# alanqrwang/nwhead

Hardware: AMD Instinct MI355X
Metric: query-predictions/sec (higher is better)
Workload: dtype f32; 1 GPU; K3 predict('full'): B=256 queries/step vs bank N=50000 d=512 C=200, bank sharded 1-way, 26 query batches coalesced per launch; B=256, N_support=50000, d=512, C=200, parallelism=support-shard x1

## Files before the change

### nwhead_amd/csrc/fused.hip

```cpp
#include <mutex>
#include <utility>
#include <vector>
#include "fused_impl.h"

namespace nw {

#define NW_EXTERN_FUSED_KIND(K) extern template int launch_fused_kind<K>(const FusedArgs&, const FusedPlan&);
NW_FOR_EACH_KIND(NW_EXTERN_FUSED_KIND)
#undef NW_EXTERN_FUSED_KIND

namespace {
struct TileTimer {
    bool on = false;
    std::vector<std::pair<hipEvent_t, hipEvent_t>> ev;
    std::vector<std::pair<hipEvent_t, hipEvent_t>> pool;
    std::mutex mu;
} g_tt;
}

int tile_timer_start(hipStream_t st) {
    if (!g_tt.on) return -1;
    std::lock_guard<std::mutex> lk(g_tt.mu);
    std::pair<hipEvent_t, hipEvent_t> p;
    if (!g_tt.pool.empty()) {
        p = g_tt.pool.back();
        g_tt.pool.pop_back();
    } else if (hipEventCreate(&p.first) != hipSuccess || hipEventCreate(&p.second) != hipSuccess) {
        return -1;
    }
    (void)hipEventRecord(p.first, st);
    g_tt.ev.push_back(p);
    return (int)g_tt.ev.size() - 1;
}
void tile_timer_stop(int slot, hipStream_t st) {
    if (slot < 0) return;
    std::lock_guard<std::mutex> lk(g_tt.mu);
    if (slot < (int)g_tt.ev.size()) (void)hipEventRecord(g_tt.ev[slot].second, st);
}
int tile_timer_enable(bool on) {
    std::lock_guard<std::mutex> lk(g_tt.mu);
    g_tt.on = on;
    return NW_OK;
}
int tile_timer_read(double* total_us, int64_t* launches) {
    std::lock_guard<std::mutex> lk(g_tt.mu);
    double tot = 0;
    for (auto& p : g_tt.ev) {
        float ms = 0.f;
        if (hipEventSynchronize(p.second) != hipSuccess || hipEventElapsedTime(&ms, p.first, p.second) != hipSuccess)
            return NW_ERR_LAUNCH;
        tot += (double)ms * 1e3;
        g_tt.pool.push_back(p);
    }
    if (total_us) *total_us = tot;
    if (launches) *launches = (int64_t)g_tt.ev.size();
    g_tt.ev.clear();
    return NW_OK;
}

namespace {
int device_cu_count() {
    static int n = [] {
        int dev = 0, v = 0;
        if (hipGetDevice(&dev) != hipSuccess) return 256;
        if (hipDeviceGetAttribute(&v, hipDeviceAttributeMultiprocessorCount, dev) != hipSuccess || v <= 0) return 256;
        return v;
    }();
    return n;
}
bool env_flag(int k) { return knob(k) == 1; }
}

inline size_t al256(size_t x) { return (x + 255) & ~(size_t)255; }

size_t fused_layout(int64_t B, int64_t n_stiles, int BS, char* base, FusedWs* ws, int64_t C) {
    size_t off = 0;
    auto take = [&](size_t bytes) {
        char* p = base ? base + off : nullptr;
        off += al256(bytes);
        return p;
    };
    FusedWs w;
    w.m = reinterpret_cast<float*>(take((size_t)n_stiles * B * 4));
    w.den = reinterpret_cast<float*>(take((size_t)n_stiles * B * 4));
    w.nrun = reinterpret_cast<int*>(take((size_t)n_stiles * 4));
    w.lab = reinterpret_cast<int*>(take((size_t)n_stiles * BS * 4));
    w.num = reinterpret_cast<float*>(take((size_t)n_stiles * BS * B * 4));
    w.runid = reinterpret_cast<int*>(take(((size_t)n_stiles * BS + 64) * 4));
    w.bnd = reinterpret_cast<int*>(take((size_t)n_stiles * 2 * 4));
    w.ctab = reinterpret_cast<int*>(take((size_t)C * (3 + 4) * 4));
    if (ws) *ws = w;
    return off;
}

namespace {

constexpr int MTHREADS = 512, MENT = 4, MTPT = 16;
template <bool PARTIAL, int MQ, int TMODE>
__global__ __launch_bounds__(MTHREADS) void nw_merge_runs_kernel(
    const float* __restrict__ ws_m, const float* __restrict__ ws_den, const int* __restrict__ ws_nrun,
    const int* __restrict__ ws_lab, const float* __restrict__ ws_num, float* __restrict__ out,
    float* __restrict__ lse, float* __restrict__ m_out, float* __restrict__ den_out,
    float* __restrict__ num_out, int B, int C, int n_stiles, int BS, const int* __restrict__ ctab) {
    constexpr bool TABLES = TMODE != 0;
    constexpr bool LTAB = TMODE == 1;
    constexpr int ML = MTHREADS / MQ;
    constexpr int MNS = MQ + 1;
    constexpr int NW = MTHREADS / 64;
    constexpr float LN2 = 0.693147180559945309417f;
    static_assert(MQ <= 32 && (MQ & (MQ - 1)) == 0, "a wave holds whole groups of MQ queries");
    extern __shared__ __attribute__((aligned(16))) char smem[];
    float* red = reinterpret_cast<float*>(smem);
    float* Ms = red + 2 * NW * MQ;
    float* inv_s = Ms + MQ;
    int* lds_tab = reinterpret_cast<int*>(inv_s + MQ);
    int* cnt = TMODE == 2 ? const_cast<int*>(ctab) : lds_tab;
    int* tlo = cnt + C;
    int* thi = tlo + C;
    int* ent = thi + C;
    float* res = reinterpret_cast<float*>(lds_tab + (size_t)C * (3 + MENT));
    const int tid = threadIdx.x, bq = tid & (MQ - 1), sl = tid / MQ, wave = tid >> 6;
    const int b0 = blockIdx.x * MQ;
    const int b = min(b0 + bq, B - 1);

    const bool in_regs = n_stiles <= ML * MTPT;
    float mr[MTPT], dr[MTPT];
    float M = -INFINITY;
    if (in_regs) {
#pragma unroll
        for (int u = 0; u < MTPT; ++u) {
            const int t = sl + u * ML;
            const bool ok = t < n_stiles;
            mr[u] = ok ? ws_m[(size_t)t * B + b] : -INFINITY;
            dr[u] = ok ? ws_den[(size_t)t * B + b] : 0.f;
        }
    }
    int tnr = 0, tl3[3] = {-1, -1, -1};
    const bool one_pass_tables = LTAB && n_stiles <= MTHREADS;
    if (one_pass_tables && tid < n_stiles) {
        tnr = ws_nrun[tid];
        const int* lt = ws_lab + (size_t)tid * BS;
        tl3[0] = lt[0];
        tl3[1] = lt[1];
        tl3[2] = lt[2];
    }
    if (LTAB) {
        for (int c = tid; c < C; c += MTHREADS) {
            cnt[c] = 0;
            tlo[c] = 0x7fffffff;
            thi[c] = -1;
        }
    }
    if (in_regs) {
#pragma unroll
        for (int u = 0; u < MTPT; ++u) M = fmaxf(M, mr[u]);
    } else {
        for (int t = sl; t < n_stiles; t += ML) M = fmaxf(M, ws_m[(size_t)t * B + b]);
    }
#pragma unroll
    for (int o = 32; o >= MQ; o >>= 1) M = fmaxf(M, __shfl_xor(M, o));
    if ((tid & 63) < MQ) red[wave * MQ + bq] = M;
    __syncthreads();
    if (LTAB) {
        auto add_tile = [&](int t, int nr, const int (&l3)[3]) {
            const int* lt = ws_lab + (size_t)t * BS;
            for (int r = 0; r < nr; ++r) {
                const int y = r < 3 ? l3[r] : lt[r];
                if (y < 0) continue;
                atomicMin(&tlo[y], t);
                atomicMax(&thi[y], t);
                const int slot = atomicAdd(&cnt[y], 1);
                if (slot < MENT) ent[y * MENT + slot] = t * BS + r;
            }
        };
        if (one_pass_tables) {
            if (tid < n_stiles) add_tile(tid, tnr, tl3);
        } else {
            for (int t = tid; t < n_stiles; t += MTHREADS) {
                const int* lt = ws_lab + (size_t)t * BS;
                const int l3[3] = {lt[0], lt[1], lt[2]};
                add_tile(t, ws_nrun[t], l3);
            }
        }
    }
    M = red[bq];
#pragma unroll
    for (int k = 1; k < NW; ++k) M = fmaxf(M, red[k * MQ + bq]);
    float den = 0.f;
    if (in_regs) {
#pragma unroll
        for (int u = 0; u < MTPT; ++u) den += dr[u] * __builtin_amdgcn_exp2f(mr[u] - M);
    } else {
        for (int t = sl; t < n_stiles; t += ML)
            den += ws_den[(size_t)t * B + b] * __builtin_amdgcn_exp2f(ws_m[(size_t)t * B + b] - M);
    }
#pragma unroll
    for (int o = 32; o >= MQ; o >>= 1) den += __shfl_xor(den, o);
    if ((tid & 63) < MQ) red[NW * MQ + wave * MQ + bq] = den;
    if (sl == 0) Ms[bq] = M;
    __syncthreads();
    if (LTAB) {
        for (int c = tid; c < C; c += MTHREADS) {
            const int n = cnt[c];
            if (n > 1 && n <= MENT) {
                int e[MENT];
#pragma unroll
                for (int k = 0; k < MENT; ++k) e[k] = k < n ? ent[c * MENT + k] : 0x7fffffff;
#pragma unroll
                for (int i = 1; i < MENT; ++i)
#pragma unroll
                    for (int j = MENT - 1; j >= i; --j)
                        if (e[j] < e[j - 1]) { const int x = e[j]; e[j] = e[j - 1]; e[j - 1] = x; }
#pragma unroll
                for (int k = 0; k < MENT; ++k)
                    if (k < n) ent[c * MENT + k] = e[k];
            }
        }
    }
    den = red[NW * MQ + bq];
#pragma unroll
    for (int k = 1; k < NW; ++k) den += red[NW * MQ + k * MQ + bq];
    if (sl == 0) inv_s[bq] = 1.f / den;
    const int nq = min(MQ, B - b0);
    if (sl == 0 && bq < nq) {
        if (PARTIAL) {
            m_out[b] = M * LN2;
            den_out[b] = den;
        } else if (lse) {
            lse[b] = M * LN2 + logf(den);
        }
    }
    __syncthreads();
    int P = 1;
    while (P < 64 && 2 * P * C * MQ <= MTHREADS) P <<= 1;
    for (int xx = tid; xx < C * MQ * P; xx += MTHREADS) {
        const int x = xx / P, sub = xx - x * P;
        const int c = x / MQ, q = x - c * MQ;
        const int bb = min(b0 + q, B - 1);
        const float Mq = Ms[q];
        float acc = 0.f;
        const int n = TABLES ? cnt[c] : MENT + 1;
        if (n <= MENT) {
            int e[MENT];
            float v[MENT], mt[MENT];
#pragma unroll
            for (int k = 0; k < MENT; ++k) e[k] = ent[c * MENT + (k < n ? k : 0)];
#pragma unroll
            for (int k = 0; k < MENT; ++k) {
                if (k < n) {
                    v[k] = ws_num[(size_t)e[k] * B + bb];
                    mt[k] = ws_m[(size_t)(e[k] / BS) * B + bb];
                }
            }
#pragma unroll
            for (int k = 0; k < MENT; ++k)
                if (k < n) acc += v[k] * __builtin_amdgcn_exp2f(mt[k] - Mq);
        } else {
            const int t0 = TABLES ? tlo[c] : 0, t1 = TABLES ? thi[c] : n_stiles - 1;
            for (int t = t0 + sub; t <= t1; t += P) {
                const int nr = ws_nrun[t];
                const float f = __builtin_amdgcn_exp2f(ws_m[(size_t)t * B + bb] - Mq);
                const int* lt = ws_lab + (size_t)t * BS;
                for (int r = 0; r < nr; ++r)
                    if (lt[r] == c) acc += ws_num[((size_t)t * BS + r) * B + bb] * f;
            }
        }
        if (P > 1) {
            if (n <= MENT && sub != 0) acc = 0.f;
            for (int o = P >> 1; o > 0; o >>= 1) acc += __shfl_xor(acc, o);
            if (sub != 0) continue;
        }
        if (LTAB && MQ > 1) {
            res[c * MNS + q] = acc;
        } else if (q < nq) {
            if (PARTIAL) num_out[(size_t)bb * C + c] = acc;
            else out[(size_t)bb * C + c] = logf(acc * inv_s[q] + NW_LOG_EPS);
        }
    }
    if (!LTAB || MQ == 1) return;
    __syncthreads();
    for (int x = tid; x < nq * C; x += MTHREADS) {
        const int qq = x / C, c = x - qq * C;
        if (PARTIAL) num_out[(size_t)(b0 + qq) * C + c] = res[c * MNS + qq];
        else out[(size_t)(b0 + qq) * C + c] = logf(res[c * MNS + qq] * inv_s[qq] + NW_LOG_EPS);
    }
}

__global__ __launch_bounds__(1024) void nw_class_tables_kernel(const int* __restrict__ ws_nrun, const int* __restrict__ ws_lab,
                                                                int n_stiles, int BS, int C, int* __restrict__ ctab) {
    int* cnt = ctab;
    int* tlo = cnt + C;
    int* thi = tlo + C;
    int* ent = thi + C;
    const int tid = threadIdx.x;
    for (int c = tid; c < C; c += 1024) {
        cnt[c] = 0;
        tlo[c] = 0x7fffffff;
        thi[c] = -1;
    }
    __threadfence();
    __syncthreads();
    for (int t = tid; t < n_stiles; t += 1024) {
        const int nr = ws_nrun[t];
        const int* lt = ws_lab + (size_t)t * BS;
        for (int r = 0; r < nr; ++r) {
            const int y = lt[r];
            if (y < 0) continue;
            atomicMin(&tlo[y], t);
            atomicMax(&thi[y], t);
            const int slot = atomicAdd(&cnt[y], 1);
            if (slot < MENT) ent[y * MENT + slot] = t * BS + r;
        }
    }
    __threadfence();
    __syncthreads();
    for (int c = tid; c < C; c += 1024) {
        const int n = cnt[c];
        if (n > 1 && n <= MENT) {
            int e[MENT];
#pragma unroll
            for (int k = 0; k < MENT; ++k) e[k] = k < n ? ent[c * MENT + k] : 0x7fffffff;
#pragma unroll
            for (int i = 1; i < MENT; ++i)
#pragma unroll
                for (int j = MENT - 1; j >= i; --j)
                    if (e[j] < e[j - 1]) { const int x = e[j]; e[j] = e[j - 1]; e[j - 1] = x; }
#pragma unroll
            for (int k = 0; k < MENT; ++k)
                if (k < n) ent[c * MENT + k] = e[k];
        }
    }
}

__global__ __launch_bounds__(64) void nw_run_tables_kernel(const int64_t* __restrict__ sy, int N, int C, int BS,
                                                           int* __restrict__ runid, int* __restrict__ nrun,
                                                           int* __restrict__ lab_out, int* __restrict__ bnd) {
    const int st = blockIdx.x, lane = threadIdx.x, s0 = st * BS;
    if (lane < 2) bnd[2 * st + lane] = BS;
    __syncthreads();
    int lab[3], flag[3];
#pragma unroll
    for (int u = 0; u < 3; ++u) {
        const int t = 3 * lane + u, j = s0 + t;
        int64_t y = -1;
        if (t < BS && j < N) y = sy[j];
        lab[u] = ((uint64_t)y < (uint64_t)C) ? (int)y : -1;
    }
    const int prev_last = __shfl_up(lab[2], 1);
    flag[0] = (lane == 0) || (lab[0] != prev_last);
    flag[1] = lab[1] != lab[0];
    flag[2] = lab[2] != lab[1];
    int incl = flag[0] + flag[1] + flag[2];
#pragma unroll
    for (int o = 1; o < 64; o <<= 1) {
        const int v = __shfl_up(incl, o);
        if (lane >= o) incl += v;
    }
    int id = incl - (flag[0] + flag[1] + flag[2]) - 1;
#pragma unroll
    for (int u = 0; u < 3; ++u) {
        const int t = 3 * lane + u;
        id += flag[u];
        if (t < BS) {
            runid[(size_t)s0 + t] = id;
            if (flag[u]) lab_out[(size_t)s0 + id] = lab[u];
            if (flag[u] && (id == 1 || id == 2)) bnd[2 * st + id - 1] = t;
            if (t == BS - 1) nrun[st] = id + 1;
        }
    }
}

int env_rs() {
    const int v = knob(KNOB_TILE_RS);
    return v == KNOB_UNSET ? 0 : v;
}

}

int query_area_of_workspace(void* workspace, size_t workspace_bytes, int64_t B, int64_t N, int64_t d, int64_t C, float** rows,
                            float** scale, float** norm2) {
    const size_t total = nw_fwd_workspace_bytes(B, N, d, C);
    if (!workspace || workspace_bytes < total) return NW_ERR_WORKSPACE;
    const size_t a = al256((size_t)B * (size_t)d * sizeof(float)), b = al256((size_t)B * sizeof(float));
    char* base = static_cast<char*>(workspace) + (total - a - 3 * b);
    *rows = reinterpret_cast<float*>(base);
    *scale = reinterpret_cast<float*>(base + a);
    *norm2 = reinterpret_cast<float*>(base + a + b);
    return NW_OK;
}

int launch_run_tables(const FusedWs& ws, const int64_t* sy, int N, int C, int n_stiles, int BS, hipStream_t st) {
    if (BS > 192) return NW_ERR_UNSUPPORTED;
    hipLaunchKernelGGL(nw_run_tables_kernel, dim3(n_stiles), dim3(64), 0, st, sy, N, C, BS, ws.runid, ws.nrun, ws.lab, ws.bnd);
    NW_CHECK_LAUNCH();
    return NW_OK;
}

constexpr int BANK_BS = 128;

size_t bank_tables_layout(int64_t n_stiles, char* base, FusedWs* ws) {
    size_t off = 0;
    auto take = [&](size_t bytes) {
        char* p = base ? base + off : nullptr;
        off += al256(bytes);
        return p;
    };
    int* nrun = reinterpret_cast<int*>(take((size_t)n_stiles * 4));
    int* lab = reinterpret_cast<int*>(take((size_t)n_stiles * BANK_BS * 4));
    int* runid = reinterpret_cast<int*>(take(((size_t)n_stiles * BANK_BS + 64) * 4));
    int* bnd = reinterpret_cast<int*>(take((size_t)n_stiles * 2 * 4));
    if (ws) {
        ws->nrun = nrun;
        ws->lab = lab;
        ws->runid = runid;
        ws->bnd = bnd;
    }
    return off;
}

bool bank_tables_take(const int64_t* sy, int N, int C, int n_stiles, int BS, FusedWs* ws) {
    (void)C;
    const FwdOpts& o = fwd_opts();
    if (!o.tables || BS != BANK_BS) return false;
    if (o.tables_sy != sy || o.tables_N != (int64_t)N) return false;
    if (o.tables_bytes < bank_tables_layout(n_stiles, nullptr, nullptr)) return false;
    bank_tables_layout(n_stiles, const_cast<char*>(o.tables), ws);
    return true;
}

int launch_merge_runs(const FusedWs& ws, float* out, float* lse, float* m, float* den, float* num,
                      int B, int C, int n_stiles, int BS, hipStream_t st) {
    auto lds_bytes = [&](int mq, bool tables) {
        return ((size_t)2 * (MTHREADS / 64) * mq + 2 * mq + (tables ? (size_t)C * (3 + MENT + mq + 1) : 0)) * sizeof(float);
    };
    const size_t cap = 150 * 1024;
    int mq = 1;
    const int force_mq = knob(KNOB_MERGE_MQ) == KNOB_UNSET ? 0 : knob(KNOB_MERGE_MQ);
    if (force_mq == 1 || force_mq == 16 || force_mq == 32) {
        mq = force_mq;
        if (lds_bytes(mq, true) > cap) mq = 1;
    } else if (B >= 512 && !env_flag(KNOB_MERGE_PER_QUERY)) {
        mq = n_stiles >= 128 ? 16 : 32;
        if (lds_bytes(mq, true) > cap) mq = 16;
        if (lds_bytes(mq, true) > cap) mq = 1;
    }
    const bool tables = lds_bytes(mq, true) <= cap;
    const size_t lds = lds_bytes(mq, tables);
    const int grid = (B + mq - 1) / mq;
#define NW_MERGE(P_, Q_, T_)                                                                                       \
    hipLaunchKernelGGL((nw_merge_runs_kernel<P_, Q_, T_>), dim3(grid), dim3(MTHREADS), lds, st, ws.m, ws.den, ws.nrun, \
                       ws.lab, ws.num, out, lse, m, den, num, B, C, n_stiles, BS, ws.ctab)
    if (!tables) {
        if (ws.ctab && !env_flag(KNOB_MERGE_NO_GLOBAL_TABLES)) {
            hipLaunchKernelGGL(nw_class_tables_kernel, dim3(1), dim3(1024), 0, st, ws.nrun, ws.lab, n_stiles, BS, C, ws.ctab);
            if (out) NW_MERGE(false, 1, 2); else NW_MERGE(true, 1, 2);
        } else {
            if (out) NW_MERGE(false, 1, 0); else NW_MERGE(true, 1, 0);
        }
    } else if (mq == 1) {
        if (out) NW_MERGE(false, 1, 1); else NW_MERGE(true, 1, 1);
    } else if (mq == 16) {
        if (out) NW_MERGE(false, 16, 1); else NW_MERGE(true, 16, 1);
    } else {
        if (out) NW_MERGE(false, 32, 1); else NW_MERGE(true, 32, 1);
    }
#undef NW_MERGE
    NW_CHECK_LAUNCH();
    return NW_OK;
}

int pick_rs(int64_t B, int64_t N, int64_t d, bool f16) {
    const int forced = env_rs();
    if (forced == 2 || forced == 4 || forced == 5 || forced == 6 || forced == 8 || forced == 10 || forced == 12)
        return forced;
    const int64_t nq = (B + BQ - 1) / BQ;
    if (forced == 0 && !f16 && d % BK == 0 && nq * ((N + 79) / 80) >= 480) return 5;
    if (forced == 0 && f16 && d % BK == 0 && nq * ((N + 127) / 128) >= 4 * 256) return 8;
    const int cand[] = {2, 4, 6, 8, 10, 12};
    const int ncand = f16 ? 5 : 6;
    double best = 1e30;
    int best_rs = 8;
    for (int ci = 0; ci < ncand; ++ci) {
        const int rs = cand[ci];
        const int64_t ns = (N + 16 * rs - 1) / (16 * rs);
        const int64_t nwg = nq * ns;
        const int64_t rounds = (nwg + 255) / 256;
        double cost = (double)rounds * (rs + 1.5);
        if (nwg >= 384) cost *= 0.85;
        if (cost < best - 1e-9) {
            best = cost;
            best_rs = rs;
        }
    }
    return best_rs;
}

bool half_form_shape_ok(int64_t d) {
    return d % 64 == 0 && d >= 192 && d <= (1 << 20);
}

namespace {
struct TileLds {
    size_t reg, dma;
    size_t p64, p64x2, p128;
};
template <int RS>
constexpr TileLds tile_lds() {
    if constexpr (RS > 5)
        return {FUSED_HDR + TileCfg<RS>::STAGE_BYTES, FUSED_HDR + DmaCfg<RS>::STAGE_BYTES, PCfg<RS, 1, false>::LDS_BYTES,
                PCfg<RS, 1, true>::LDS_BYTES, PCfg<RS, 2, false>::LDS_BYTES};
    else
        return {FUSED_HDR + TileCfg<RS>::STAGE_BYTES, FUSED_HDR + DmaCfg<RS>::STAGE_BYTES, 0, 0, 0};
}
TileLds tile_lds_of(int rs) {
    return rs == 2 ? tile_lds<2>() : rs == 4 ? tile_lds<4>() : rs == 5 ? tile_lds<5>() : rs == 6 ? tile_lds<6>()
         : rs == 8 ? tile_lds<8>() : rs == 10 ? tile_lds<10>() : tile_lds<12>();
}
}

FusedPlan plan_tiles(int64_t B, int64_t N, int64_t d, int form) {
    FusedPlan p = {};
    p.form = form;
    p.rs = form == FORM_HALF ? BANK_BS / 16 : pick_rs(B, N, d, form == FORM_SPLIT);
    p.BS = 16 * p.rs;
    const int64_t n_stiles = (N + p.BS - 1) / p.BS, n_qtiles = (B + BQ - 1) / BQ;
    const int64_t grid = (n_stiles + 7) / 8 * 8 * n_qtiles;
    if (grid > 0x7fffffff) p.status = NW_ERR_UNSUPPORTED;
    else p.n_stiles = (int)n_stiles, p.n_qtiles = (int)n_qtiles, p.grid = (int)grid;
    return p;
}

FusedPlan plan_fused(int64_t B, int64_t N, int64_t d, int64_t C, int form, int out, int k, bool norms, bool dot, int cus,
                     const FwdOpts& opts) {
    (void)C; (void)k;
    if (B < 0 || N < 0 || d < 0 || B >= (1 << 30) || N >= (1 << 30) || d >= (1 << 30)) {
        FusedPlan none = {};
        return none.status = NW_ERR_UNSUPPORTED, none;
    }
    FusedPlan p = plan_tiles(B, N, d, form);
    if (p.status != NW_OK) return p;
    auto refuse = [&p](int status) { p.status = status; return p; };
    if (cus <= 0) cus = device_cu_count();
    const TileLds lds = tile_lds_of(p.rs);
    const bool split = form == FORM_SPLIT;
    p.out = out;
    p.dma = (d % BK) == 0 && (uint64_t)(BQ + p.BS) * 2 * d * 4 < 0xffffffffull;
    if (form == FORM_HALF) {
        if (out != OUT_NONE || !half_form_shape_ok(d)) return refuse(NW_ERR_UNSUPPORTED);
        p.persistent = true;
    } else {
        if (!p.dma && (p.rs & 1)) return refuse(NW_ERR_UNSUPPORTED);
        p.persistent = split && out == OUT_NONE && p.rs > 5 && (p.rs == 8 || env_flag(KNOB_PERSISTENT_ANY_RS)) &&
                       p.grid >= 4 * (int64_t)cus && d >= 3 * BK && !env_flag(KNOB_NO_PERSISTENT);
    }
    p.run_tables = p.persistent;
    if (p.run_tables && p.BS > 192) return refuse(NW_ERR_UNSUPPORTED);
    if (split && (!p.dma || !norms)) return refuse(NW_ERR_INVALID_ARG);
    if (out == OUT_CAND && !split) return refuse(NW_ERR_INVALID_ARG);
    if (out == OUT_CAND && p.rs == 12) return refuse(NW_ERR_UNSUPPORTED);
    if (p.persistent) {
        p.mode = MODE_F16;
        p.split_queries = true;
        int wgs = cus & ~7;
        const int wg_cap = opts.persistent_wgs & ~7;
        if (wg_cap >= 8 && wg_cap < wgs) wgs = wg_cap;
        int variant = form == FORM_HALF ? 3 : knob(KNOB_PVAR);
        if (variant < 0 || variant > 3) {
            const double rows64 = 1.15 * ((B + 63) / 64 * 64);
            variant = (p.rs == 8 && (B + 255) / 256 * 256 <= rows64) ? 3 : ((B + 127) / 128 * 128 <= rows64) ? 2 : 1;
        }
        if (variant == 3 && p.rs != 8) variant = 2;
        if (variant == 2 && lds.p128 > 160 * 1024) variant = 0;
        if (variant == 1 && lds.p64x2 > 80 * 1024) variant = 0;
        p.variant = variant;
        p.workgroups = variant == 1 ? 2 * wgs : wgs;
        const int qg = (knob(KNOB_QG) >= 1 && knob(KNOB_QG) <= 64) ? knob(KNOB_QG) : 8;
        p.qgroup = variant != 3 ? qg : qg >= 2 ? qg / 2 : 1;
        p.lds_bytes = variant == 3 ? (size_t)P12::LDS_BYTES : variant == 2 ? lds.p128 : variant == 1 ? lds.p64x2 : lds.p64;
        return p;
    }
    if (split) {
        const int force_split = knob(KNOB_SPLIT_QUERIES) == KNOB_UNSET ? -1 : knob(KNOB_SPLIT_QUERIES);
        const bool raw_ok = force_split == 0 || (force_split < 0 && 2 * (int64_t)p.grid <= 3 * (int64_t)cus);
        p.split_queries = !raw_ok;
        p.mode = raw_ok ? MODE_F16Q : MODE_F16;
    } else {
        p.mode = !p.dma ? MODE_REG : (norms && !dot) ? MODE_DMA_SN : MODE_DMA;
    }
    p.lds_bytes = p.mode == MODE_REG ? lds.reg : lds.dma;
    return p;
}

size_t fused_workspace_bytes(int64_t B, int64_t N, int64_t d, int64_t C) {
    size_t need = 0;
    for (int form : {FORM_F32, FORM_SPLIT, FORM_HALF}) {
        if (form == FORM_HALF && !half_form_shape_ok(d)) continue;
        const int BS = plan_tiles(B, N, d, form).BS;
        const size_t n = fused_layout(B, (N + BS - 1) / BS, BS, nullptr, nullptr, C);
        need = n > need ? n : need;
    }
    return need;
}

bool fused_eligible(const float* q, const float* s, int64_t B, int64_t N, int64_t d, int64_t C) {
    const bool aligned = ((reinterpret_cast<uintptr_t>(q) | reinterpret_cast<uintptr_t>(s)) & 15) == 0;
    return N > 25 && d >= 4 && (d % 4) == 0 && aligned && B < (1 << 30) && N < (1 << 30) &&
           d < (1 << 30) && C < (1 << 30) && (8 + C) * 4 <= 160 * 1024;
}

int launch_fused(const FusedArgs& a, int form, int kind) {
    const int out = a.cand ? OUT_CAND : a.scores ? OUT_SCORES : OUT_NONE;
    const FusedPlan p = plan_fused(a.B, a.N, a.d, a.C, form, out, a.cand ? a.cand->k : 0, a.s_norm2 != nullptr,
                                   kind == NW_SCORE_DOT, 0, fwd_opts());
#define NW_KIND_CASE(K) case K: return launch_fused_kind<K>(a, p);
    switch (kind) {
        NW_FOR_EACH_KIND(NW_KIND_CASE)
        default: return NW_ERR_UNSUPPORTED;
    }
#undef NW_KIND_CASE
}

namespace {
struct KnnWs {
    CandOut cand;
    int64_t n_stiles;
    int kcp;
};
bool knn_shape_ok(int64_t B, int64_t N, int64_t d, int64_t k) {
    return B >= 0 && N > 25 && d >= BK && d % BK == 0 && k >= 1 && k <= 32 && k <= N && B < (1 << 30) && N < (1 << 30) &&
           d <= (1 << 20);
}
size_t knn_layout(int64_t B, int64_t N, int64_t d, int64_t k, int BS, char* base, KnnWs* out) {
    KnnWs w;
    w.n_stiles = (N + BS - 1) / BS;
    w.kcp = cand_slots((int)k, BS);
    size_t off = 0;
    auto take = [&](size_t bytes) {
        char* p = base ? base + off : nullptr;
        off += al256(bytes);
        return p;
    };
    const size_t slots = (size_t)B * (size_t)w.n_stiles * (size_t)w.kcp;
    w.cand.key = reinterpret_cast<unsigned*>(take(slots * 4));
    w.cand.row = reinterpret_cast<int*>(take(slots * 4));
    w.cand.q_rows = reinterpret_cast<float*>(take((size_t)B * (size_t)d * 4));
    w.cand.q_scale = reinterpret_cast<float*>(take((size_t)B * 4));
    w.cand.q_norm2 = reinterpret_cast<float*>(take((size_t)B * 4));
    w.cand.k = (int)k;
    if (out) *out = w;
    return off;
}
}

size_t knn_workspace_bytes(int64_t B, int64_t N, int64_t d, int64_t k) {
    if (!knn_shape_ok(B, N, d, k) || B == 0) return 0;
    if (pick_rs(B, N, d, true) > 10) return 0;
    size_t need = knn_layout(B, N, d, k, 16 * pick_rs(B, N, d, true), nullptr, nullptr);
    const int64_t nq = (B + BQ - 1) / BQ;
    for (int64_t qt = 1; qt <= nq && qt < 1024; ++qt) {
        const int64_t Bq = qt * BQ < B ? qt * BQ : B;
        for (int64_t n = 17; n <= N && qt * ((n + 127) / 128) < 1024; n += 16) {
            const int64_t nn = n > 26 ? n : 26;
            if (nn > N || k > nn) continue;
            const size_t x = knn_layout(Bq, nn, d, k, 16 * pick_rs(Bq, nn, d, true), nullptr, nullptr);
            need = x > need ? x : need;
        }
    }
    return need;
}

int launch_knn(const float* q, const float* s_split, const float* s_scale, const float* s_norm2, int64_t* idx, float* vals,
               void* workspace, size_t workspace_bytes, int64_t B, int64_t N, int64_t d, int64_t k, int kind, const float* ls,
               hipStream_t st) {
    if (!knn_shape_ok(B, N, d, k)) return NW_ERR_UNSUPPORTED;
    if (B == 0) return NW_OK;
    KnnWs w;
    const size_t need = knn_layout(B, N, d, k, plan_tiles(B, N, d, FORM_SPLIT).BS, static_cast<char*>(workspace), &w);
    if (!workspace || workspace_bytes < need) return NW_ERR_WORKSPACE;
    if (w.n_stiles * w.kcp >= (1ll << 31)) return NW_ERR_UNSUPPORTED;
    FusedArgs a = {};
    a.q = q, a.s = s_split, a.s_norm2 = s_norm2, a.s_scale = s_scale, a.ls = ls;
    a.B = (int)B, a.N = (int)N, a.d = (int)d, a.C = 1, a.st = st, a.cand = &w.cand;
    const int rc = launch_fused(a, FORM_SPLIT, kind);
    if (rc != NW_OK) return rc;
    return launch_topk_candidates(w.cand.key, w.cand.row, idx, vals, B, w.n_stiles * w.kcp, k, st);
}

}

extern "C" size_t nw_bank_tables_bytes(int64_t N) {
    if (N <= 0 || N > 0x7fffffffLL) return 0;
    return nw::bank_tables_layout((N + nw::BANK_BS - 1) / nw::BANK_BS, nullptr, nullptr);
}

extern "C" int nw_bank_tables_build(const int64_t* sy, int64_t N, int64_t C, void* tables, size_t tables_bytes,
                                    void* stream) {
    using namespace nw;
    if (N < 0 || C < 0 || N > 0x7fffffffLL || C > 0x7fffffffLL) return NW_ERR_INVALID_ARG;
    if (N == 0) return NW_OK;
    if (!sy || !tables || (reinterpret_cast<uintptr_t>(tables) & 15)) return NW_ERR_INVALID_ARG;
    const int64_t n_stiles = (N + BANK_BS - 1) / BANK_BS;
    FusedWs ws;
    if (tables_bytes < bank_tables_layout(n_stiles, static_cast<char*>(tables), &ws)) return NW_ERR_WORKSPACE;
    return launch_run_tables(ws, sy, (int)N, (int)C, (int)n_stiles, BANK_BS, static_cast<hipStream_t>(stream));
}
```

Baseline: 7.821 million query-predictions/s.

## Batch merge gathers across classes and cache per-tile maxima in LDS

Adds a dedicated path for the merge kernel when each class item has a single worker (P==1). Each thread gathers the numerator and tile-max loads for MCH items up front, with scheduling barriers, so many global loads are in flight before the exp/accumulate step. Per-tile maxima are staged in LDS when they fit, and class-table entries are re-encoded as (tile<<8|run), replacing the divide by BS with shifts and masks. In exchange the kernel uses more registers and LDS (launch bounds now request 4 blocks), and launches with BS>256 are rejected as unsupported.

```diff
diff --git a/nwhead_amd/csrc/fused.hip b/nwhead_amd/csrc/fused.hip
--- a/nwhead_amd/csrc/fused.hip
+++ b/nwhead_amd/csrc/fused.hip
@@ -95,13 +95,14 @@
 
 namespace {
 
-constexpr int MTHREADS = 512, MENT = 4, MTPT = 16;
+constexpr int MTHREADS = 512, MENT = 4, MTPT = 16, MCH = 8;
+constexpr int ENT_SH = 8, ENT_RUN = (1 << ENT_SH) - 1;
 template <bool PARTIAL, int MQ, int TMODE>
-__global__ __launch_bounds__(MTHREADS) void nw_merge_runs_kernel(
+__global__ __launch_bounds__(MTHREADS, 4) void nw_merge_runs_kernel(
     const float* __restrict__ ws_m, const float* __restrict__ ws_den, const int* __restrict__ ws_nrun,
     const int* __restrict__ ws_lab, const float* __restrict__ ws_num, float* __restrict__ out,
     float* __restrict__ lse, float* __restrict__ m_out, float* __restrict__ den_out,
-    float* __restrict__ num_out, int B, int C, int n_stiles, int BS, const int* __restrict__ ctab) {
+    float* __restrict__ num_out, int B, int C, int n_stiles, int BS, const int* __restrict__ ctab, int mts_off) {
     constexpr bool TABLES = TMODE != 0;
     constexpr bool LTAB = TMODE == 1;
     constexpr int ML = MTHREADS / MQ;
@@ -119,6 +120,8 @@
     int* thi = tlo + C;
     int* ent = thi + C;
     float* res = reinterpret_cast<float*>(lds_tab + (size_t)C * (3 + MENT));
+    float* mts = reinterpret_cast<float*>(smem) + (mts_off < 0 ? 0 : mts_off);
+    const bool mt_lds = mts_off >= 0;
     const int tid = threadIdx.x, bq = tid & (MQ - 1), sl = tid / MQ, wave = tid >> 6;
     const int b0 = blockIdx.x * MQ;
     const int b = min(b0 + bq, B - 1);
@@ -133,6 +136,13 @@
             const bool ok = t < n_stiles;
             mr[u] = ok ? ws_m[(size_t)t * B + b] : -INFINITY;
             dr[u] = ok ? ws_den[(size_t)t * B + b] : 0.f;
+        }
+        if (mt_lds) {
+#pragma unroll
+            for (int u = 0; u < MTPT; ++u) {
+                const int t = sl + u * ML;
+                if (t < n_stiles) mts[t * MQ + bq] = mr[u];
+            }
         }
     }
     int tnr = 0, tl3[3] = {-1, -1, -1};
@@ -170,7 +180,7 @@
                 atomicMin(&tlo[y], t);
                 atomicMax(&thi[y], t);
                 const int slot = atomicAdd(&cnt[y], 1);
-                if (slot < MENT) ent[y * MENT + slot] = t * BS + r;
+                if (slot < MENT) ent[y * MENT + slot] = t << ENT_SH | r;
             }
         };
         if (one_pass_tables) {
@@ -233,6 +243,68 @@
     __syncthreads();
     int P = 1;
     while (P < 64 && 2 * P * C * MQ <= MTHREADS) P <<= 1;
+    if (TABLES && P == 1) {
+        const int items = C * MQ;
+        const unsigned last_tile = n_stiles - 1, last_row = (unsigned)n_stiles * BS - 1;
+        const float* mt_src = mt_lds ? mts : ws_m;
+        const size_t mt_stride = mt_lds ? (size_t)MQ : (size_t)B;
+        for (int x0 = tid; x0 < items; x0 += MCH * MTHREADS) {
+            int cj[MCH], nj[MCH], bj[MCH];
+            unsigned ej[MCH][MENT];
+#pragma unroll
+            for (int j = 0; j < MCH; ++j) {
+                const int x = x0 + j * MTHREADS;
+                const int c = x < items ? x / MQ : 0;
+                cj[j] = c;
+                nj[j] = cnt[c];
+                bj[j] = min(b0 + (x & (MQ - 1)), B - 1);
+#pragma unroll
+                for (int k = 0; k < MENT; ++k) ej[j][k] = (unsigned)ent[c * MENT + k];
+            }
+            auto tile_of = [&](unsigned e) { return min(e >> ENT_SH, last_tile); };
+            auto row_of = [&](unsigned e) { return min(tile_of(e) * (unsigned)BS + (e & ENT_RUN), last_row); };
+            float v[MCH][MENT], mt[MCH][MENT];
+#pragma unroll
+            for (int j = 0; j < MCH; ++j) {
+                const size_t mo = mt_lds ? (size_t)((x0 + j * MTHREADS) & (MQ - 1)) : (size_t)bj[j];
+#pragma unroll
+                for (int k = 0; k < MENT; ++k) v[j][k] = ws_num[(size_t)row_of(ej[j][k]) * B + bj[j]];
+#pragma unroll
+                for (int k = 0; k < MENT; ++k) mt[j][k] = mt_src[(size_t)tile_of(ej[j][k]) * mt_stride + mo];
+                __builtin_amdgcn_sched_barrier(0);
+            }
+#pragma unroll
+            for (int j = 0; j < MCH; ++j) {
+                const int x = x0 + j * MTHREADS;
+                if (x >= items) break;
+                const int c = cj[j], q = x & (MQ - 1), n = nj[j];
+                const float Mq = Ms[q];
+                float acc = 0.f;
+#pragma unroll
+                for (int k = 0; k < MENT; ++k) {
+                    const float a = acc + v[j][k] * __builtin_amdgcn_exp2f(mt[j][k] - Mq);
+                    acc = k < n ? a : acc;
+                }
+                if (n > MENT) {
+                    acc = 0.f;
+                    const int bb = bj[j];
+                    for (int t = tlo[c]; t <= thi[c]; ++t) {
+                        const int nr = ws_nrun[t];
+                        const float f = __builtin_amdgcn_exp2f(ws_m[(size_t)t * B + bb] - Mq);
+                        const int* lt = ws_lab + (size_t)t * BS;
+                        for (int r = 0; r < nr; ++r)
+                            if (lt[r] == c) acc += ws_num[((size_t)t * BS + r) * B + bb] * f;
+                    }
+                }
+                if (LTAB && MQ > 1) {
+                    res[c * MNS + q] = acc;
+                } else if (q < nq) {
+                    if (PARTIAL) num_out[(size_t)bj[j] * C + c] = acc;
+                    else out[(size_t)bj[j] * C + c] = logf(acc * inv_s[q] + NW_LOG_EPS);
+                }
+            }
+        }
+    } else
     for (int xx = tid; xx < C * MQ * P; xx += MTHREADS) {
         const int x = xx / P, sub = xx - x * P;
         const int c = x / MQ, q = x - c * MQ;
@@ -248,8 +320,8 @@
 #pragma unroll
             for (int k = 0; k < MENT; ++k) {
                 if (k < n) {
-                    v[k] = ws_num[(size_t)e[k] * B + bb];
-                    mt[k] = ws_m[(size_t)(e[k] / BS) * B + bb];
+                    v[k] = ws_num[(size_t)((e[k] >> ENT_SH) * BS + (e[k] & ENT_RUN)) * B + bb];
+                    mt[k] = ws_m[(size_t)(e[k] >> ENT_SH) * B + bb];
                 }
             }
 #pragma unroll
@@ -309,7 +381,7 @@
             atomicMin(&tlo[y], t);
             atomicMax(&thi[y], t);
             const int slot = atomicAdd(&cnt[y], 1);
-            if (slot < MENT) ent[y * MENT + slot] = t * BS + r;
+            if (slot < MENT) ent[y * MENT + slot] = t << ENT_SH | r;
         }
     }
     __threadfence();
@@ -434,6 +506,7 @@
         return ((size_t)2 * (MTHREADS / 64) * mq + 2 * mq + (tables ? (size_t)C * (3 + MENT + mq + 1) : 0)) * sizeof(float);
     };
     const size_t cap = 150 * 1024;
+    if (BS > ENT_RUN + 1 || n_stiles > (0x7fffffff >> ENT_SH)) return NW_ERR_UNSUPPORTED;
     int mq = 1;
     const int force_mq = knob(KNOB_MERGE_MQ) == KNOB_UNSET ? 0 : knob(KNOB_MERGE_MQ);
     if (force_mq == 1 || force_mq == 16 || force_mq == 32) {
@@ -445,11 +518,16 @@
         if (lds_bytes(mq, true) > cap) mq = 1;
     }
     const bool tables = lds_bytes(mq, true) <= cap;
-    const size_t lds = lds_bytes(mq, tables);
+    size_t lds = lds_bytes(mq, tables);
+    int mts_off = -1;
+    if (n_stiles <= (MTHREADS / mq) * MTPT && lds + (size_t)n_stiles * mq * sizeof(float) <= cap) {
+        mts_off = (int)(lds / sizeof(float));
+        lds += (size_t)n_stiles * mq * sizeof(float);
+    }
     const int grid = (B + mq - 1) / mq;
 #define NW_MERGE(P_, Q_, T_)                                                                                       \
     hipLaunchKernelGGL((nw_merge_runs_kernel<P_, Q_, T_>), dim3(grid), dim3(MTHREADS), lds, st, ws.m, ws.den, ws.nrun, \
-                       ws.lab, ws.num, out, lse, m, den, num, B, C, n_stiles, BS, ws.ctab)
+                       ws.lab, ws.num, out, lse, m, den, num, B, C, n_stiles, BS, ws.ctab, mts_off)
     if (!tables) {
         if (ws.ctab && !env_flag(KNOB_MERGE_NO_GLOBAL_TABLES)) {
             hipLaunchKernelGGL(nw_class_tables_kernel, dim3(1), dim3(1024), 0, st, ws.nrun, ws.lab, n_stiles, BS, C, ws.ctab);
```

Result: no change. 7.798 million query-predictions/s (-0.3%).
